# Distributed-Learning-Networking-Group/torchgpipe

Hardware: AMD Instinct MI355X
Metric: U-Net(5,64) GPipe training throughput (samples/sec) (higher is better)
Workload: dtype fp32; 1 GPU; model=U-Net(5,64), experiment=pipeline-1, global_batch=80, input=3x192x192, chunks=2, checkpoint=except_last, parallelism=pp1, transport=none, fused_cells=True, cell_streams=0, overlap_recompute=True, overlap_forward=True, graph_cells=False, hw_queues=4

## Files before the change

### torchgpipe_amd/csrc/bindings.cpp

```cpp
#include <algorithm>
#include <torch/extension.h>
#include <ATen/hip/HIPContext.h>
#include <ATen/hip/impl/HIPGuardImplMasqueradingAsCUDA.h>

#include <vector>

#include "kernels.h"

namespace tgpipe {
namespace {

hipStream_t stream_of(const at::Tensor& t) {
  return at::hip::getCurrentHIPStream(t.device().index()).stream();
}

const int64_t* rng_state(const c10::optional<at::Tensor>& rng, const at::Device& device) {
  if (!rng.has_value() || !rng->defined()) return nullptr;
  TORCH_CHECK(rng->is_cuda() && rng->device() == device && rng->scalar_type() == at::kLong &&
                  rng->is_contiguous() && rng->numel() == 2,
              "rng must be a contiguous int64 [2] (seed, offset) tensor on the op's device");
  return rng->data_ptr<int64_t>();
}

void check_f32_gpu(const at::Tensor& t, const char* name) {
  TORCH_CHECK(t.is_cuda(), name, " must be a GPU tensor");
  TORCH_CHECK(t.scalar_type() == at::kFloat, name, " must be float32");
  TORCH_CHECK(t.is_contiguous(), name, " must be contiguous");
}

std::vector<at::Tensor> dna_forward(const at::Tensor& x, double p, double eps, double slope,
                                    int64_t seed, int64_t offset, bool dropout,
                                    const c10::optional<at::Tensor>& rng) {
  check_f32_gpu(x, "x");
  TORCH_CHECK(x.dim() >= 3, "expected (N, C, *spatial) input");
  TORCH_CHECK(p >= 0.0 && p < 1.0, "dropout probability must be in [0, 1)");
  const int64_t planes = x.size(0) * x.size(1);
  const int64_t s = planes == 0 ? 0 : x.numel() / planes;
  c10::hip::HIPGuardMasqueradingAsCUDA guard(x.device());
  auto y = at::empty_like(x);
  auto opts = x.options();
  auto mean = at::empty({planes}, opts);
  auto rstd = at::empty({planes}, opts);
  auto scale = at::empty({planes}, opts);
  launch_dna_forward(x.data_ptr<float>(), y.data_ptr<float>(), mean.data_ptr<float>(),
                     rstd.data_ptr<float>(), scale.data_ptr<float>(), planes, s,
                     static_cast<float>(p), static_cast<float>(eps), static_cast<float>(slope),
                     static_cast<uint64_t>(seed), static_cast<uint64_t>(offset), dropout,
                     rng_state(rng, x.device()), stream_of(x));
  return {y, mean, rstd, scale};
}

at::Tensor dna_backward(const at::Tensor& dy_in, const at::Tensor& x, const at::Tensor& mean,
                        const at::Tensor& rstd, const at::Tensor& scale, double slope) {
  check_f32_gpu(x, "x");
  auto dy = dy_in.contiguous();
  check_f32_gpu(dy, "dy");
  TORCH_CHECK(dy.sizes() == x.sizes(), "dy and x must have the same shape");
  const int64_t planes = x.size(0) * x.size(1);
  const int64_t s = planes == 0 ? 0 : x.numel() / planes;
  TORCH_CHECK(mean.numel() == planes && rstd.numel() == planes && scale.numel() == planes,
              "saved statistics must have N*C elements");
  c10::hip::HIPGuardMasqueradingAsCUDA guard(x.device());
  auto dx = at::empty_like(x);
  launch_dna_backward(dy.data_ptr<float>(), x.data_ptr<float>(), mean.data_ptr<float>(),
                      rstd.data_ptr<float>(), scale.data_ptr<float>(), dx.data_ptr<float>(),
                      planes, s, static_cast<float>(slope), stream_of(x));
  return dx;
}

at::Tensor dropout(const at::Tensor& x_in, double p, int64_t seed, int64_t offset,
                   const c10::optional<at::Tensor>& rng) {
  auto x = x_in.contiguous();
  check_f32_gpu(x, "x");
  TORCH_CHECK(p >= 0.0 && p < 1.0, "dropout probability must be in [0, 1)");
  c10::hip::HIPGuardMasqueradingAsCUDA guard(x.device());
  auto y = at::empty_like(x);
  launch_dropout(x.data_ptr<float>(), y.data_ptr<float>(), x.numel(), static_cast<float>(p),
                 static_cast<uint64_t>(seed), static_cast<uint64_t>(offset),
                 rng_state(rng, x.device()), stream_of(x));
  return y;
}

at::Tensor philox_uniform(int64_t n, int64_t seed, int64_t offset, at::Device device,
                          const c10::optional<at::Tensor>& rng) {
  TORCH_CHECK(device.is_cuda(), "philox_uniform runs on the GPU");
  c10::hip::HIPGuardMasqueradingAsCUDA guard(device);
  auto out = at::empty({n}, at::TensorOptions().dtype(at::kFloat).device(device));
  launch_philox_uniform(out.data_ptr<float>(), n, static_cast<uint64_t>(seed),
                        static_cast<uint64_t>(offset), rng_state(rng, out.device()),
                        stream_of(out));
  return out;
}

void spin(int64_t ns, at::Device device) {
  TORCH_CHECK(device.is_cuda(), "spin runs on the GPU");
  c10::hip::HIPGuardMasqueradingAsCUDA guard(device);
  launch_spin(static_cast<uint64_t>(ns),
              at::hip::getCurrentHIPStream(device.index()).stream());
}

void copy_segments(at::TensorList srcs, at::TensorList dsts) {
  TORCH_CHECK(srcs.size() == dsts.size(), "srcs and dsts must pair up");
  if (srcs.empty()) return;
  const auto device = srcs[0].device();
  TORCH_CHECK(device.is_cuda(), "copy_segments runs on the GPU");
  c10::hip::HIPGuardMasqueradingAsCUDA guard(device);
  std::vector<Segment> segs;
  for (size_t i = 0; i < srcs.size(); ++i) {
    TORCH_CHECK(srcs[i].is_contiguous() && dsts[i].is_contiguous(), "segments must be contiguous");
    TORCH_CHECK(srcs[i].device() == device && dsts[i].device() == device,
                "segments must live on one device");
    const int64_t bytes = srcs[i].numel() * srcs[i].element_size();
    TORCH_CHECK(bytes == dsts[i].numel() * dsts[i].element_size(), "segment size mismatch");
    segs.push_back({srcs[i].data_ptr(), dsts[i].data_ptr(), bytes});
  }
  const hipStream_t stream = at::hip::getCurrentHIPStream(device.index()).stream();
  for (size_t i = 0; i < segs.size(); i += kMaxSegments) {
    const int count = static_cast<int>(std::min<size_t>(kMaxSegments, segs.size() - i));
    launch_segments_copy(segs.data() + i, count, stream);
  }
}

at::Tensor transform_out(const c10::optional<at::Tensor>& out, at::IntArrayRef shape,
                         const at::Tensor& like) {
  if (!out.has_value() || !out->defined()) return at::empty(shape, like.options());
  check_f32_gpu(*out, "out");
  TORCH_CHECK(out->sizes() == shape && out->device() == like.device(),
              "out must be the transform's shape on the weight's device");
  return *out;
}

at::Tensor wino_weight(const at::Tensor& w, bool flip, const c10::optional<at::Tensor>& out) {
  check_f32_gpu(w, "weight");
  TORCH_CHECK(w.dim() == 4 && w.size(2) == 3 && w.size(3) == 3, "weight must be [K][C][3][3]");
  const int64_t out_channels = flip ? w.size(1) : w.size(0);
  const int64_t red_channels = flip ? w.size(0) : w.size(1);
  c10::hip::HIPGuardMasqueradingAsCUDA guard(w.device());
  auto u = transform_out(
      out, {wino_pad_reduction(red_channels), wino_pad_output(out_channels), 16}, w);
  launch_wino_weight(w.data_ptr<float>(), u.data_ptr<float>(), out_channels, red_channels, flip,
                     stream_of(w));
  return u;
}

at::Tensor wino_conv(const at::Tensor& x_in, const at::Tensor& u,
                     const c10::optional<at::Tensor>& bias, int64_t out_channels,
                     int64_t variant, int64_t splits) {
  auto x = x_in.contiguous();
  check_f32_gpu(x, "x");
  check_f32_gpu(u, "u");
  TORCH_CHECK(x.dim() == 4, "x must be NCHW");
  const int64_t n = x.size(0), r = x.size(1), h = x.size(2), w = x.size(3);
  TORCH_CHECK(u.dim() == 3 && u.size(2) == 16 && u.size(0) == wino_pad_reduction(r) &&
                  u.size(1) == wino_pad_output(out_channels),
              "transformed weight does not match the input/output channels");
  TORCH_CHECK(u.device() == x.device(), "u must live on the input's device");
  TORCH_CHECK(n * ((h + 1) / 2) * ((w + 1) / 2) < (int64_t{1} << 31) * 32,
              "too many output tiles for one launch");
  TORCH_CHECK(r * h * w < (int64_t{1} << 31) && out_channels < (1 << 24),
              "plane too large for 32-bit channel offsets");
  const float* bptr = nullptr;
  if (bias.has_value() && bias->defined()) {
    check_f32_gpu(*bias, "bias");
    TORCH_CHECK(bias->numel() == out_channels, "bias must have K elements");
    bptr = bias->data_ptr<float>();
  }
  c10::hip::HIPGuardMasqueradingAsCUDA guard(x.device());
  TORCH_CHECK(variant >= -1 && variant <= 2, "variant must be -1 (auto), 0, 1 or 2");
  auto y = at::empty({n, out_channels, h, w}, x.options());
  if (y.numel() == 0) return y;
  const WinoPlan plan = wino_plan(n, r, h, w, out_channels, static_cast<int>(variant),
                                  static_cast<int>(splits));
  at::Tensor ws;
  if (plan.workspace > 0) ws = at::empty({plan.workspace}, x.options());
  launch_wino_conv(x.data_ptr<float>(), u.data_ptr<float>(), bptr, y.data_ptr<float>(),
                   plan.workspace > 0 ? ws.data_ptr<float>() : nullptr, n, r, h, w, out_channels,
                   plan, stream_of(x));
  return y;
}

at::Tensor wino4_weight(const at::Tensor& w, bool flip, const c10::optional<at::Tensor>& out) {
  check_f32_gpu(w, "weight");
  TORCH_CHECK(w.dim() == 4 && w.size(2) == 3 && w.size(3) == 3, "weight must be [K][C][3][3]");
  const int64_t out_channels = flip ? w.size(1) : w.size(0);
  const int64_t red_channels = flip ? w.size(0) : w.size(1);
  c10::hip::HIPGuardMasqueradingAsCUDA guard(w.device());
  auto u = transform_out(
      out, {wino4_pad_reduction(red_channels), wino4_pad_output(out_channels), 36}, w);
  launch_wino4_weight(w.data_ptr<float>(), u.data_ptr<float>(), out_channels, red_channels, flip,
                      stream_of(w));
  return u;
}

std::vector<int64_t> wino4_emu_weight_shape(int64_t out_channels, int64_t red_channels) {
  return {wino4_emu_pad_reduction(red_channels) / 16, wino4_pad_output(out_channels) / 64, 36,
          1024};
}

at::Tensor wino4_weight_emu(const at::Tensor& w, bool flip,
                            const c10::optional<at::Tensor>& out) {
  check_f32_gpu(w, "weight");
  TORCH_CHECK(w.dim() == 4 && w.size(2) == 3 && w.size(3) == 3, "weight must be [K][C][3][3]");
  const int64_t out_channels = flip ? w.size(1) : w.size(0);
  const int64_t red_channels = flip ? w.size(0) : w.size(1);
  c10::hip::HIPGuardMasqueradingAsCUDA guard(w.device());
  const auto wc = w.contiguous();
  auto u = transform_out(out, wino4_emu_weight_shape(out_channels, red_channels), w);
  TORCH_CHECK(u.is_contiguous(), "out must be contiguous");
  if (u.numel() == 0) return u;
  launch_wino4_emu_weight(wc.data_ptr<float>(), u.data_ptr<float>(), out_channels, red_channels,
                          flip, stream_of(w));
  return u;
}

at::Tensor wino4_conv(const at::Tensor& x_in, const at::Tensor& u,
                      const c10::optional<at::Tensor>& bias, int64_t out_channels,
                      int64_t variant, int64_t splits) {
  auto x = x_in.contiguous();
  check_f32_gpu(x, "x");
// ... 63 lines not shown
  auto dw = wgrad_destination(into, x, k, c);
  if (n == 0 || h == 0 || w == 0) return accum ? dw : dw.zero_();
  TORCH_CHECK(variant == -1 || variant == 0 || variant == 2, "variant must be -1, 0 or 2");
  const int64_t tiles = n * ((h + 1) / 2) * ((w + 1) / 2);
  int v = variant >= 0 ? static_cast<int>(variant) : (k <= 32 ? 0 : 2);
  if (v == 2 && tiles >= (int64_t{1} << 24)) v = 0;
  const int64_t steps = (tiles + 7) / 8;
  const int s = static_cast<int>(std::min<int64_t>(
      splits > 0 ? splits : wino_wgrad_splits(n, c, k, h, w, v), steps));
  at::Tensor ws;
  if (s > 1) ws = at::empty({s * k * c * 9}, x.options());
  launch_wino_wgrad(x.data_ptr<float>(), dy.data_ptr<float>(), dw.data_ptr<float>(),
                    s > 1 ? ws.data_ptr<float>() : nullptr, n, c, k, h, w, s, v, accum,
                    stream_of(x));
  return dw;
}

at::Tensor wino4_wgrad(const at::Tensor& x_in, const at::Tensor& dy_in, int64_t splits,
                       int64_t variant, const c10::optional<at::Tensor>& into) {
  auto x = x_in.contiguous();
  auto dy = dy_in.contiguous();
  check_f32_gpu(x, "x");
  check_f32_gpu(dy, "dy");
  TORCH_CHECK(x.dim() == 4 && dy.dim() == 4, "x and dy must be NCHW");
  const int64_t n = x.size(0), c = x.size(1), h = x.size(2), w = x.size(3), k = dy.size(1);
  TORCH_CHECK(dy.size(0) == n && dy.size(2) == h && dy.size(3) == w,
              "dy must be [N][K][H][W] of a 3x3/s1/p1 convolution of x");
  TORCH_CHECK(dy.device() == x.device(), "x and dy must share a device");
  c10::hip::HIPGuardMasqueradingAsCUDA guard(x.device());
  const bool accum = into.has_value();
  auto dw = wgrad_destination(into, x, k, c);
  if (n == 0 || h == 0 || w == 0 || c == 0 || k == 0) return accum ? dw : dw.zero_();
  TORCH_CHECK(wino4_wgrad_supported(n, c, k, h, w),
              "input too large for the F(4x4) weight-gradient kernel (needs < 1 GiB); "
              "use wino_wgrad");
  TORCH_CHECK(variant >= 0 && variant <= 3,
              "variant must be 0 (fused), 1 (non-fused), 2 (split-bf16 batched GEMM) or 3 (fused, "
              "x rows through LDS)");
  const WinoPlan plan = wino4_wgrad_plan(n, c, k, h, w, static_cast<int>(variant),
                                         static_cast<int>(splits));
  at::Tensor ws;
  if (plan.workspace > 0) ws = at::empty({plan.workspace}, x.options());
  launch_wino4_wgrad(x.data_ptr<float>(), dy.data_ptr<float>(), dw.data_ptr<float>(),
                     plan.workspace > 0 ? ws.data_ptr<float>() : nullptr, n, c, k, h, w, plan,
                     accum, stream_of(x));
  return dw;
}

at::Tensor bg_weight(const at::Tensor& w, bool flip, int64_t kind,
                     const c10::optional<at::Tensor>& out, int64_t emu) {
  check_f32_gpu(w, "weight");
  TORCH_CHECK(w.dim() == 4 && w.size(2) == 3 && w.size(3) == 3, "weight must be [K][C][3][3]");
  auto wc = w.contiguous();
  const int64_t out_channels = flip ? w.size(1) : w.size(0);
  const int64_t red_channels = flip ? w.size(0) : w.size(1);
  c10::hip::HIPGuardMasqueradingAsCUDA guard(w.device());
  TORCH_CHECK(kind == 4 || kind == 2, "kind must be 4 (F(4x4)) or 2 (F(2x2))");
  auto a =
      transform_out(out, {bg_weight_numel(out_channels, red_channels, static_cast<int>(kind),
                                          static_cast<int>(emu))}, w);
  launch_bg_weight(wc.data_ptr<float>(), a.data_ptr<float>(), out_channels, red_channels, flip,
                   static_cast<int>(kind), stream_of(w), static_cast<int>(emu));
  return a;
}

at::Tensor bg_conv(const at::Tensor& x_in, const at::Tensor& a,
                   const c10::optional<at::Tensor>& bias, int64_t out_channels, int64_t bn,
                   int64_t splits, int64_t kind, int64_t waves, int64_t sub, int64_t emu,
                   const c10::optional<at::Tensor>& stats) {
  auto x = x_in.contiguous();
  check_f32_gpu(x, "x");
  check_f32_gpu(a, "a");
  TORCH_CHECK(x.dim() == 4, "x must be NCHW");
  const int64_t n = x.size(0), r = x.size(1), h = x.size(2), w = x.size(3);
  TORCH_CHECK(kind == 4 || kind == 2, "kind must be 4 (F(4x4)) or 2 (F(2x2))");
  TORCH_CHECK(a.dim() == 1 && a.numel() == bg_weight_numel(out_channels, r, static_cast<int>(kind),
                                                           static_cast<int>(emu)),
              "batched-GEMM transformed weight does not match the input/output channels");
  TORCH_CHECK(a.device() == x.device(), "a must live on the input's device");
  TORCH_CHECK(wino4_supported(n, r, h, w, out_channels),
              "input too large for the F(4x4) kernels (needs < 1 GiB)");
  const float* bptr = nullptr;
  if (bias.has_value() && bias->defined()) {
    check_f32_gpu(*bias, "bias");
    TORCH_CHECK(bias->numel() == out_channels, "bias must have K elements");
    bptr = bias->data_ptr<float>();
  }
  c10::hip::HIPGuardMasqueradingAsCUDA guard(x.device());
  auto y = at::empty({n, out_channels, h, w}, x.options());
  if (n == 0 || h == 0 || w == 0 || out_channels == 0) return y;
  const BgPlan plan = bg_plan(n, r, h, w, out_channels, static_cast<int>(bn),
                              static_cast<int>(splits), static_cast<int>(kind),
                              static_cast<int>(waves), static_cast<int>(sub),
                              static_cast<int>(emu));
  TORCH_CHECK(plan.ksteps * 16 * plan.np < (int64_t{1} << 31) &&
                  plan.mp * plan.np < (int64_t{1} << 31),
              "operands too large for the batched-GEMM kernels");
  float* pm = nullptr;
  int ipg = 0;
  if (stats.has_value() && stats->defined()) {
    check_f32_gpu(*stats, "stats");
    ipg = bg_stats_ipg(n, h, w, static_cast<int>(kind));
    const int64_t groups = (n + ipg - 1) / ipg;
    TORCH_CHECK(stats->device() == x.device() && stats->is_contiguous() &&
                    stats->numel() == 2 * groups * out_channels,
                "stats must be a contiguous [2][ceil(n / bg_stats_ipg)][K] float32 tensor");
    pm = stats->data_ptr<float>();
  }
  auto ws = at::empty({plan.workspace}, x.options());
  launch_bg_conv(x.data_ptr<float>(), a.data_ptr<float>(), bptr, y.data_ptr<float>(),
                 ws.data_ptr<float>(), n, r, h, w, out_channels, plan, stream_of(x), pm,
                 pm == nullptr ? nullptr : pm + stats->numel() / 2, ipg);
  return y;
}

int64_t bg_stats_images(int64_t n, int64_t h, int64_t w, int64_t kind) {
  return bg_stats_ipg(n, h, w, static_cast<int>(kind));
}

int64_t wino4_splits(int64_t n, int64_t c, int64_t k, int64_t h, int64_t w, int64_t variant) {
  if (variant == 0) return wino4_wgrad_plan(n, c, k, h, w, 0, 0).splits;
  return wino4_plan(n, c, h, w, k, static_cast<int>(variant), 0).splits;
}

std::vector<int64_t> wino4_plan_info(int64_t n, int64_t c, int64_t k, int64_t h, int64_t w,
                                     int64_t variant, int64_t splits) {
  const WinoPlan p = wino4_plan(n, c, h, w, k, static_cast<int>(variant),
                                static_cast<int>(splits));
  return {p.variant, p.og, p.splits, p.workspace};
}

std::vector<int64_t> wino4_wgrad_plan_info(int64_t n, int64_t c, int64_t k, int64_t h, int64_t w,
                                           int64_t variant, int64_t splits) {
  const WinoPlan p = wino4_wgrad_plan(n, c, k, h, w, static_cast<int>(variant),
                                      static_cast<int>(splits));
  return {p.variant, p.splits, p.workspace};
}

std::vector<int64_t> bg_plan_info(int64_t n, int64_t c, int64_t k, int64_t h, int64_t w,
                                  int64_t bn, int64_t splits, int64_t kind, int64_t waves,
                                  int64_t sub, int64_t emu) {
  const BgPlan p = bg_plan(n, c, h, w, k, static_cast<int>(bn), static_cast<int>(splits),
                           static_cast<int>(kind), static_cast<int>(waves),
                           static_cast<int>(sub), static_cast<int>(emu));
  return {p.kind, p.emu ? 1 : 0, p.waves, p.bn, p.sub, p.splits, p.ksteps, p.mp, p.np,
          p.workspace};
}

}
}

TORCH_LIBRARY(tgpipe, m) {
  m.def("dna_forward(Tensor x, float p, float eps, float slope, int seed, int offset, "
        "bool dropout, Tensor? rng=None) -> Tensor[]");
  m.def("dna_backward(Tensor dy, Tensor x, Tensor mean, Tensor rstd, Tensor scale, "
        "float slope) -> Tensor");
  m.def("dropout(Tensor x, float p, int seed, int offset, Tensor? rng=None) -> Tensor");
  m.def("philox_uniform(int n, int seed, int offset, Device device, Tensor? rng=None) -> Tensor");
  m.def("spin(int ns, Device device) -> ()");
  m.def("copy_segments(Tensor[] srcs, Tensor(a!)[] dsts) -> ()");
  m.def("wino_weight(Tensor w, bool flip, Tensor? out=None) -> Tensor");
  m.def("wino_wgrad(Tensor x, Tensor dy, int splits=0, int variant=-1, Tensor? into=None) -> Tensor");
  m.def("wino_conv(Tensor x, Tensor u, Tensor? bias, int out_channels, int variant=-1, "
        "int splits=0) -> Tensor");
  m.def("wino4_weight(Tensor w, bool flip, Tensor? out=None) -> Tensor");
  m.def("wino4_weight_emu(Tensor w, bool flip, Tensor? out=None) -> Tensor");
  m.def("wino4_wgrad(Tensor x, Tensor dy, int splits=0, int variant=0, Tensor? into=None) -> Tensor");
  m.def("wino4_conv(Tensor x, Tensor u, Tensor? bias, int out_channels, int variant=-1, "
        "int splits=0) -> Tensor");
  m.def("bg_weight(Tensor w, bool flip, int kind=4, Tensor? out=None, int emu=-1) -> Tensor");
  m.def("wino4_splits(int n, int c, int k, int h, int w, int variant) -> int",
        &tgpipe::wino4_splits);
  m.def("bg_conv(Tensor x, Tensor a, Tensor? bias, int out_channels, int bn=0, int splits=0, "
        "int kind=4, int waves=0, int sub=0, int emu=-1, Tensor(b!)? stats=None) -> Tensor");
  m.def("wino4_plan_info(int n, int c, int k, int h, int w, int variant, int splits) -> int[]",
        &tgpipe::wino4_plan_info);
  m.def("wino4_wgrad_plan_info(int n, int c, int k, int h, int w, int variant, int splits) "
        "-> int[]", &tgpipe::wino4_wgrad_plan_info);
  m.def("bg_plan_info(int n, int c, int k, int h, int w, int bn, int splits, int kind, "
        "int waves, int sub, int emu) -> int[]", &tgpipe::bg_plan_info);
  m.def("bg_stats_images(int n, int h, int w, int kind) -> int", &tgpipe::bg_stats_images);
}

TORCH_LIBRARY_IMPL(tgpipe, CUDA, m) {
  m.impl("dna_forward", &tgpipe::dna_forward);
  m.impl("dna_backward", &tgpipe::dna_backward);
  m.impl("dropout", &tgpipe::dropout);
  m.impl("copy_segments", &tgpipe::copy_segments);
  m.impl("wino_weight", &tgpipe::wino_weight);
  m.impl("wino_conv", &tgpipe::wino_conv);
  m.impl("wino_wgrad", &tgpipe::wino_wgrad);
  m.impl("wino4_weight", &tgpipe::wino4_weight);
  m.impl("wino4_weight_emu", &tgpipe::wino4_weight_emu);
  m.impl("wino4_conv", &tgpipe::wino4_conv);
  m.impl("wino4_wgrad", &tgpipe::wino4_wgrad);
  m.impl("bg_weight", &tgpipe::bg_weight);
  m.impl("bg_conv", &tgpipe::bg_conv);
}

TORCH_LIBRARY_IMPL(tgpipe, CompositeExplicitAutograd, m) {
  m.impl("philox_uniform", &tgpipe::philox_uniform);
  m.impl("spin", &tgpipe::spin);
}

PYBIND11_MODULE(TORCH_EXTENSION_NAME, m) {
  m.doc() = "torchgpipe_amd native HIP kernels (gfx950)";
}
```

### torchgpipe_amd/csrc/kernels.h

```cpp
#pragma once
#include <hip/hip_runtime.h>
#include <stdint.h>

#include <vector>

namespace tgpipe {

void launch_dna_forward(const float* x, float* y, float* mean, float* rstd, float* scale,
                        int64_t planes, int64_t s, float p, float eps, float slope,
                        uint64_t seed, uint64_t offset, bool dropout, const int64_t* rng,
                        hipStream_t stream);

void launch_dna_backward(const float* dy, const float* x, const float* mean, const float* rstd,
                         const float* scale, float* dx, int64_t planes, int64_t s, float slope,
                         hipStream_t stream);

void launch_dropout(const float* x, float* y, int64_t n, float p, uint64_t seed, uint64_t offset,
                    const int64_t* rng, hipStream_t stream);

void launch_philox_uniform(float* out, int64_t n, uint64_t seed, uint64_t offset,
                           const int64_t* rng, hipStream_t stream);

void launch_spin(uint64_t ns, hipStream_t stream);

struct Segment {
  const void* src;
  void* dst;
  int64_t bytes;
};
constexpr int kMaxSegments = 16;
void launch_segments_copy(const Segment* segs, int count, hipStream_t stream);

int64_t wino_pad_reduction(int64_t r);
int64_t wino_pad_output(int64_t o);
void launch_wino_weight(const float* w, float* u, int64_t out_channels, int64_t red_channels,
                        bool flip, hipStream_t stream);
struct WinoPlan {
  int variant = 0;
  int splits = 1;
  int64_t workspace = 0;
  int og = 0;
};
WinoPlan wino_plan(int64_t n, int64_t red_channels, int64_t h, int64_t w, int64_t out_channels,
                   int variant, int splits);
void launch_wino_conv(const float* x, const float* u, const float* bias, float* y, float* ws,
                      int64_t n, int64_t red_channels, int64_t h, int64_t w, int64_t out_channels,
                      const WinoPlan& plan, hipStream_t stream);

int64_t wino4_pad_reduction(int64_t r);
int64_t wino4_pad_output(int64_t o);
bool wino4_supported(int64_t n, int64_t r, int64_t h, int64_t w, int64_t o);
void launch_wino4_weight(const float* w, float* u, int64_t out_channels, int64_t red_channels,
                         bool flip, hipStream_t stream);
bool wino4_variant_known(int variant);
bool wino4_variant_emu(int variant);
int64_t wino4_emu_pad_reduction(int64_t r);
int64_t wino4_emu_weight_numel(int64_t out_channels, int64_t red_channels);
void launch_wino4_emu_weight(const float* w, float* u, int64_t out_channels,
                             int64_t red_channels, bool flip, hipStream_t stream);
WinoPlan wino4_plan(int64_t n, int64_t red_channels, int64_t h, int64_t w, int64_t out_channels,
                    int variant, int splits);
void launch_wino4_conv(const float* x, const float* u, const float* bias, float* y, float* ws,
                       int64_t n, int64_t red_channels, int64_t h, int64_t w, int64_t out_channels,
                       const WinoPlan& plan, hipStream_t stream);

struct BgPlan {
  int kind = 4;
  int waves = 8;
  int bn = 64;
  int sub = 1;
  int splits = 1;
  bool emu = false;
  int64_t mp = 0, np = 0, ksteps = 0;
  int64_t workspace = 0;
};
bool bg_emu(int emu);
int bg_pick_bn(int64_t tiles, int kind, bool emu = false);
BgPlan bg_plan(int64_t n, int64_t red_channels, int64_t h, int64_t w, int64_t out_channels,
               int bn, int splits, int kind, int waves, int sub, int emu = -1);
int64_t bg_weight_numel(int64_t out_channels, int64_t red_channels, int kind, int emu = -1);
void launch_bg_weight(const float* w, float* a, int64_t out_channels, int64_t red_channels,
                      bool flip, int kind, hipStream_t stream, int emu = -1);
int bg_stats_ipg(int64_t n, int64_t h, int64_t w, int kind);
void launch_bg_conv(const float* x, const float* a, const float* bias, float* y, float* ws,
                    int64_t n, int64_t red_channels, int64_t h, int64_t w, int64_t out_channels,
                    const BgPlan& plan, hipStream_t stream, float* pm = nullptr,
                    float* pm2 = nullptr, int ipg = 0);


bool wino4_wgrad_supported(int64_t n, int64_t c, int64_t k, int64_t h, int64_t w);
WinoPlan wino4_wgrad_plan(int64_t n, int64_t c, int64_t k, int64_t h, int64_t w, int variant,
                          int splits);
void launch_wino4_wgrad(const float* x, const float* dy, float* dw, float* ws, int64_t n,
                        int64_t c, int64_t k, int64_t h, int64_t w, const WinoPlan& plan,
                        bool accum, hipStream_t stream);

int wino_wgrad_splits(int64_t n, int64_t c, int64_t k, int64_t h, int64_t w, int variant);
void launch_wino_wgrad(const float* x, const float* dy, float* dw, float* ws, int64_t n,
                       int64_t c, int64_t k, int64_t h, int64_t w, int splits, int variant,
                       bool accum, hipStream_t stream);


struct ConvGemmTail {
  const float* gamma = nullptr;
  const float* beta = nullptr;
  const float* mean = nullptr;
  const float* var = nullptr;
  const float* add = nullptr;
  float eps = 0.f;
  int relu_out = 0;
};
struct ConvGemmGeo {
  int n, ci, h, w;
  int co, ho, wo;
  int co_total, co_off;
  int kh, kw, sh, sw, ph, pw;
  int oh, ow;
  bool relu;
  bool a_t = false;
  bool phase = false;
  int zh = 0, zw = 0, dy0 = 0, dx0 = 0;
  bool fill = false;
  bool a_split = false;
  ConvGemmTail tail;
};
struct ConvGemmPhase {
  ConvGemmGeo geo;
  int th0, tw0;
};
bool conv_gemm_phased(const ConvGemmGeo& g);
constexpr int kConvGemmMaxPhases = 4;
struct ConvGemmPlan;
void launch_conv_gemm_phases(const float* a, const int64_t* a_off, const float* b,
                             const float* x_mask, float* out, const ConvGemmPhase* phases,
                             int count, const ConvGemmPlan& plan, bool accumulate,
                             int64_t a_bytes, int64_t b_bytes, hipStream_t stream);
int env_int(const char* name, int fallback);
std::vector<ConvGemmPhase> conv_gemm_phases(const ConvGemmGeo& g);
struct ConvGemmPlan {
  int cfg = 1;
  int splits = 1;
  int col_width = 128;
  int col_blocks = 0;
  bool scatter = false;
};
ConvGemmPlan conv_gemm_plan(int mode, const ConvGemmGeo& g);
std::vector<ConvGemmPlan> conv_gemm_candidates(int mode, const ConvGemmGeo& g);
int64_t conv_gemm_workspace(int mode, const ConvGemmGeo& g, const ConvGemmPlan& plan);
void launch_conv_gemm(int mode, const float* a, const float* b, const float* x_mask, float* out,
                      float* part_mean, float* part_m2, const ConvGemmGeo& g,
                      const ConvGemmPlan& plan, bool accumulate, float* ws, int64_t a_bytes,
                      int64_t b_bytes, hipStream_t stream);
bool conv_gemm_emu_cfg(int cfg);
int conv_precision(int level);
int conv_precision_level();
class ConvPrecisionPin {
 public:
  explicit ConvPrecisionPin(int level);
  ~ConvPrecisionPin();
  ConvPrecisionPin(const ConvPrecisionPin&) = delete;
  ConvPrecisionPin& operator=(const ConvPrecisionPin&) = delete;

 private:
  int saved_;
};
void launch_conv_gemm_presplit(const float* w, void* out, int M, int K, int taps,
                               bool transposed, hipStream_t stream);
void launch_conv_gemm_wgrad_slab(const float* a, const float* b, float* slab,
// ... 94 lines not shown
```

### torchgpipe_amd/csrc/kernels.hip

```cpp
#include "kernels.h"
#include "philox.h"

#include <hip/hip_runtime.h>
#include <math.h>

namespace tgpipe {

namespace {

constexpr int kWave = 64;

__device__ __forceinline__ float wave_sum(float v) {
#pragma unroll
  for (int o = kWave / 2; o > 0; o >>= 1) v += __shfl_xor(v, o, kWave);
  return v;
}

template <int GROUP>
__device__ __forceinline__ float group_sum_in_wave(float v) {
#pragma unroll
  for (int o = GROUP / 2; o > 0; o >>= 1) v += __shfl_xor(v, o, kWave);
  return v;
}

inline int ceil_div(int64_t a, int64_t b) { return static_cast<int>((a + b - 1) / b); }

template <int GROUP>
constexpr int kPlaneBlock = GROUP >= 256 ? GROUP : 256;

template <int GROUP, int V, bool VEC>
struct PlaneTile {
  static constexpr int kBlock = kPlaneBlock<GROUP>;
  static constexpr int kPlanesPerBlock = kBlock / GROUP;
  static constexpr int kCap = GROUP * V * 4;

  __device__ static __forceinline__ int64_t index(int t, int k, int j) {
    return VEC ? static_cast<int64_t>(k * GROUP + t) * 4 + j
               : static_cast<int64_t>(k * 4 + j) * GROUP + t;
  }

  __device__ static __forceinline__ void load(const float* __restrict__ p, int t, int64_t s,
                                              bool active, float (&r)[V * 4]) {
#pragma unroll
    for (int k = 0; k < V; ++k) {
      if (VEC) {
        const int64_t idx = index(t, k, 0);
        float4 v = (active && idx < s) ? *reinterpret_cast<const float4*>(p + idx)
                                       : make_float4(0, 0, 0, 0);
        r[k * 4 + 0] = v.x;
        r[k * 4 + 1] = v.y;
        r[k * 4 + 2] = v.z;
        r[k * 4 + 3] = v.w;
      } else {
#pragma unroll
        for (int j = 0; j < 4; ++j) {
          const int64_t idx = index(t, k, j);
          r[k * 4 + j] = (active && idx < s) ? p[idx] : 0.f;
        }
      }
    }
  }

  __device__ static __forceinline__ void store(float* __restrict__ p, int t, int64_t s,
                                               bool active, const float (&r)[V * 4]) {
    if (!active) return;
#pragma unroll
    for (int k = 0; k < V; ++k) {
      if (VEC) {
        const int64_t idx = index(t, k, 0);
        if (idx < s)
          *reinterpret_cast<float4*>(p + idx) =
              make_float4(r[k * 4 + 0], r[k * 4 + 1], r[k * 4 + 2], r[k * 4 + 3]);
      } else {
#pragma unroll
        for (int j = 0; j < 4; ++j) {
          const int64_t idx = index(t, k, j);
          if (idx < s) p[idx] = r[k * 4 + j];
        }
      }
    }
  }

  __device__ static __forceinline__ bool valid(int t, int k, int j, int64_t s) {
    return index(t, k, j) < s;
  }

  __device__ static __forceinline__ float reduce(float v, float* lds) {
    if (GROUP <= kWave) return group_sum_in_wave<GROUP>(v);
    v = wave_sum(v);
    const int wave = threadIdx.x / kWave;
    if ((threadIdx.x & (kWave - 1)) == 0) lds[wave] = v;
    __syncthreads();
    float total = 0.f;
#pragma unroll
    for (int w = 0; w < GROUP / kWave; ++w) total += lds[w];
    __syncthreads();
    return total;
  }
};

__device__ __forceinline__ void philox_resolve(const int64_t* __restrict__ rng, uint64_t& seed,
                                               uint64_t& offset) {
  if (rng != nullptr) {
    seed = static_cast<uint64_t>(rng[0]);
    offset += static_cast<uint64_t>(rng[1]);
  }
}

__device__ __forceinline__ float plane_dropout_scale(int64_t plane, float p, uint64_t seed,
                                                     uint64_t offset, bool dropout) {
  if (!dropout) return 1.f;
  const float u = philox_uniform(philox4x32_10(static_cast<uint64_t>(plane), offset, seed).v[0]);
  return u >= p ? 1.f / (1.f - p) : 0.f;
}

template <int GROUP, int V, bool VEC>
__global__ __launch_bounds__(kPlaneBlock<GROUP>) void dna_forward_kernel(
    const float* __restrict__ x, float* __restrict__ y, float* __restrict__ mean_out,
    float* __restrict__ rstd_out, float* __restrict__ scale_out, int64_t planes, int64_t s,
    float p, float eps, float slope, uint64_t seed, uint64_t offset, bool dropout,
    const int64_t* __restrict__ rng) {
  using T = PlaneTile<GROUP, V, VEC>;
  philox_resolve(rng, seed, offset);
  __shared__ float lds[T::kBlock / kWave];
  const int t = threadIdx.x % GROUP;
  const int64_t plane = static_cast<int64_t>(blockIdx.x) * T::kPlanesPerBlock + threadIdx.x / GROUP;
  const bool active = plane < planes;
  const float* xp = x + (active ? plane : 0) * s;

  float r[V * 4];
  T::load(xp, t, s, active, r);

  float acc = 0.f;
#pragma unroll
  for (int e = 0; e < V * 4; ++e) acc += r[e];
  const float inv_s = 1.f / static_cast<float>(s);
  const float mean = T::reduce(acc, lds) * inv_s;

  float sq = 0.f;
#pragma unroll
  for (int k = 0; k < V; ++k)
#pragma unroll
    for (int j = 0; j < 4; ++j) {
      const float d = T::valid(t, k, j, s) ? r[k * 4 + j] - mean : 0.f;
      sq += d * d;
    }
  const float var = T::reduce(sq, lds) * inv_s;

  const float scale = plane_dropout_scale(plane, p, seed, offset, dropout);
  const float rstd = rsqrtf(scale * scale * var + eps);
  const float mul = scale * rstd;
#pragma unroll
  for (int e = 0; e < V * 4; ++e) {
    const float z = (r[e] - mean) * mul;
    r[e] = z > 0.f ? z : z * slope;
  }
  T::store(y + (active ? plane : 0) * s, t, s, active, r);
  if (active && t == 0) {
    mean_out[plane] = mean;
    rstd_out[plane] = rstd;
    scale_out[plane] = scale;
  }
}

template <int GROUP, int V, bool VEC>
__global__ __launch_bounds__(kPlaneBlock<GROUP>) void dna_backward_kernel(
    const float* __restrict__ dy, const float* __restrict__ x, const float* __restrict__ mean_in,
    const float* __restrict__ rstd_in, const float* __restrict__ scale_in, float* __restrict__ dx,
    int64_t planes, int64_t s, float slope) {
  using T = PlaneTile<GROUP, V, VEC>;
  __shared__ float lds[T::kBlock / kWave];
  const int t = threadIdx.x % GROUP;
  const int64_t plane = static_cast<int64_t>(blockIdx.x) * T::kPlanesPerBlock + threadIdx.x / GROUP;
  const bool active = plane < planes;
  const int64_t base = (active ? plane : 0) * s;

  const float mean = active ? mean_in[plane] : 0.f;
  const float rstd = active ? rstd_in[plane] : 0.f;
  const float scale = active ? scale_in[plane] : 0.f;
  const float mul = scale * rstd;

  float z[V * 4];
  float g[V * 4];
  T::load(x + base, t, s, active, z);
  T::load(dy + base, t, s, active, g);

  float sg = 0.f, sgz = 0.f;
#pragma unroll
  for (int e = 0; e < V * 4; ++e) {
    z[e] = (z[e] - mean) * mul;
    g[e] = z[e] > 0.f ? g[e] : g[e] * slope;
    sg += g[e];
    sgz += g[e] * z[e];
  }
  const float inv_s = 1.f / static_cast<float>(s);
  const float mg = T::reduce(sg, lds) * inv_s;
  const float mgz = T::reduce(sgz, lds) * inv_s;
#pragma unroll
  for (int e = 0; e < V * 4; ++e) g[e] = mul * (g[e] - mg - z[e] * mgz);
  T::store(dx + base, t, s, active, g);
}

constexpr int kBigGroup = 1024;

__global__ __launch_bounds__(kBigGroup) void dna_forward_big_kernel(
    const float* __restrict__ x, float* __restrict__ y, float* __restrict__ mean_out,
    float* __restrict__ rstd_out, float* __restrict__ scale_out, int64_t s, float p, float eps,
    float slope, uint64_t seed, uint64_t offset, bool dropout, const int64_t* __restrict__ rng) {
  __shared__ float lds[kBigGroup / kWave];
  philox_resolve(rng, seed, offset);
  using T = PlaneTile<kBigGroup, 1, false>;
  const int64_t plane = blockIdx.x;
  const float* xp = x + plane * s;
  float acc = 0.f;
  for (int64_t i = threadIdx.x; i < s; i += kBigGroup) acc += xp[i];
  const float inv_s = 1.f / static_cast<float>(s);
  const float mean = T::reduce(acc, lds) * inv_s;
  float sq = 0.f;
  for (int64_t i = threadIdx.x; i < s; i += kBigGroup) {
    const float d = xp[i] - mean;
    sq += d * d;
  }
  const float var = T::reduce(sq, lds) * inv_s;
  const float scale = plane_dropout_scale(plane, p, seed, offset, dropout);
  const float rstd = rsqrtf(scale * scale * var + eps);
  const float mul = scale * rstd;
  float* yp = y + plane * s;
  for (int64_t i = threadIdx.x; i < s; i += kBigGroup) {
    const float z = (xp[i] - mean) * mul;
    yp[i] = z > 0.f ? z : z * slope;
  }
  if (threadIdx.x == 0) {
    mean_out[plane] = mean;
    rstd_out[plane] = rstd;
    scale_out[plane] = scale;
  }
}

__global__ __launch_bounds__(kBigGroup) void dna_backward_big_kernel(
    const float* __restrict__ dy, const float* __restrict__ x, const float* __restrict__ mean_in,
    const float* __restrict__ rstd_in, const float* __restrict__ scale_in, float* __restrict__ dx,
    int64_t s, float slope) {
  __shared__ float lds[kBigGroup / kWave];
  using T = PlaneTile<kBigGroup, 1, false>;
  const int64_t plane = blockIdx.x;
  const float mean = mean_in[plane];
  const float mul = scale_in[plane] * rstd_in[plane];
  const float* xp = x + plane * s;
  const float* gp = dy + plane * s;
  float sg = 0.f, sgz = 0.f;
  for (int64_t i = threadIdx.x; i < s; i += kBigGroup) {
    const float z = (xp[i] - mean) * mul;
    const float g = z > 0.f ? gp[i] : gp[i] * slope;
    sg += g;
    sgz += g * z;
  }
  const float inv_s = 1.f / static_cast<float>(s);
  const float mg = T::reduce(sg, lds) * inv_s;
  const float mgz = T::reduce(sgz, lds) * inv_s;
  float* dp = dx + plane * s;
  for (int64_t i = threadIdx.x; i < s; i += kBigGroup) {
    const float z = (xp[i] - mean) * mul;
    const float g = z > 0.f ? gp[i] : gp[i] * slope;
    dp[i] = mul * (g - mg - z * mgz);
  }
}

__global__ __launch_bounds__(256) void dropout_kernel(const float* __restrict__ x,
                                                      float* __restrict__ y, int64_t n, float p,
                                                      uint64_t seed, uint64_t offset, bool vec,
                                                      const int64_t* __restrict__ rng) {
  philox_resolve(rng, seed, offset);
  const float scale = 1.f / (1.f - p);
  const int64_t quads = (n + 3) / 4;
  for (int64_t q = static_cast<int64_t>(blockIdx.x) * blockDim.x + threadIdx.x; q < quads;
       q += static_cast<int64_t>(gridDim.x) * blockDim.x) {
    const PhiloxOut r = philox4x32_10(static_cast<uint64_t>(q), offset, seed);
    const int64_t e0 = q * 4;
    if (vec && e0 + 3 < n) {
      float4 v = *reinterpret_cast<const float4*>(x + e0);
      v.x = philox_uniform(r.v[0]) >= p ? v.x * scale : 0.f;
      v.y = philox_uniform(r.v[1]) >= p ? v.y * scale : 0.f;
      v.z = philox_uniform(r.v[2]) >= p ? v.z * scale : 0.f;
      v.w = philox_uniform(r.v[3]) >= p ? v.w * scale : 0.f;
      *reinterpret_cast<float4*>(y + e0) = v;
    } else {
      for (int j = 0; j < 4 && e0 + j < n; ++j)
        y[e0 + j] = philox_uniform(r.v[j]) >= p ? x[e0 + j] * scale : 0.f;
    }
  }
}

__global__ __launch_bounds__(256) void philox_uniform_kernel(float* __restrict__ out, int64_t n,
                                                             uint64_t seed, uint64_t offset,
                                                             const int64_t* __restrict__ rng) {
  philox_resolve(rng, seed, offset);
  const int64_t quads = (n + 3) / 4;
  for (int64_t q = static_cast<int64_t>(blockIdx.x) * blockDim.x + threadIdx.x; q < quads;
       q += static_cast<int64_t>(gridDim.x) * blockDim.x) {
    const PhiloxOut r = philox4x32_10(static_cast<uint64_t>(q), offset, seed);
    for (int j = 0; j < 4 && q * 4 + j < n; ++j) out[q * 4 + j] = philox_uniform(r.v[j]);
  }
}

__global__ void spin_kernel(uint64_t ticks) {
  const uint64_t t0 = __builtin_amdgcn_s_memrealtime();
  const uint64_t limit = ticks < 6000000000ull ? ticks : 6000000000ull;
  while (__builtin_amdgcn_s_memrealtime() - t0 < limit) __builtin_amdgcn_s_sleep(8);
}

struct SegmentTable {
  Segment seg[kMaxSegments];
};

__global__ __launch_bounds__(256) void segments_copy_kernel(SegmentTable table) {
  const Segment sg = table.seg[blockIdx.y];
  const uintptr_t a = reinterpret_cast<uintptr_t>(sg.src) | reinterpret_cast<uintptr_t>(sg.dst);
  const int64_t stride = static_cast<int64_t>(gridDim.x) * blockDim.x;
  const int64_t tid = static_cast<int64_t>(blockIdx.x) * blockDim.x + threadIdx.x;
  if ((a & 15) == 0) {
    const int64_t nvec = sg.bytes / 16;
    const uint4* s = reinterpret_cast<const uint4*>(sg.src);
    uint4* d = reinterpret_cast<uint4*>(sg.dst);
    for (int64_t i = tid; i < nvec; i += stride) d[i] = s[i];
    const int64_t tail = nvec * 16;
    const char* sb = reinterpret_cast<const char*>(sg.src);
    char* db = reinterpret_cast<char*>(sg.dst);
    for (int64_t i = tail + tid; i < sg.bytes; i += stride) db[i] = sb[i];
  } else {
    const char* sb = reinterpret_cast<const char*>(sg.src);
    char* db = reinterpret_cast<char*>(sg.dst);
    for (int64_t i = tid; i < sg.bytes; i += stride) db[i] = sb[i];
  }
}

template <int GROUP, int V, bool VEC>
void dna_fwd_launch(const float* x, float* y, float* mean, float* rstd, float* scale,
                    int64_t planes, int64_t s, float p, float eps, float slope, uint64_t seed,
                    uint64_t offset, bool dropout, const int64_t* rng, hipStream_t stream) {
  using T = PlaneTile<GROUP, V, VEC>;
  const int grid = ceil_div(planes, T::kPlanesPerBlock);
  hipLaunchKernelGGL((dna_forward_kernel<GROUP, V, VEC>), dim3(grid), dim3(T::kBlock), 0, stream,
                     x, y, mean, rstd, scale, planes, s, p, eps, slope, seed, offset, dropout,
                     rng);
}

template <int GROUP, int V, bool VEC>
void dna_bwd_launch(const float* dy, const float* x, const float* mean, const float* rstd,
                    const float* scale, float* dx, int64_t planes, int64_t s, float slope,
                    hipStream_t stream) {
  using T = PlaneTile<GROUP, V, VEC>;
  const int grid = ceil_div(planes, T::kPlanesPerBlock);
  hipLaunchKernelGGL((dna_backward_kernel<GROUP, V, VEC>), dim3(grid), dim3(T::kBlock), 0,
                     stream, dy, x, mean, rstd, scale, dx, planes, s, slope);
}

#define TGPIPE_DNA_DISPATCH(LAUNCH, VEC, ...)                      \
  if (s <= 16 * 1 * 4) {                                           \
    LAUNCH<16, 1, VEC>(__VA_ARGS__);                               \
  } else if (s <= 64 * 1 * 4) {                                    \
    LAUNCH<64, 1, VEC>(__VA_ARGS__);                               \
  } else if (s <= 64 * 3 * 4) {                                    \
    LAUNCH<64, 3, VEC>(__VA_ARGS__);                               \
  } else if (s <= 64 * 9 * 4) {                                    \
    LAUNCH<64, 9, VEC>(__VA_ARGS__);                               \
  } else if (s <= 256 * 9 * 4) {                                   \
    LAUNCH<256, 9, VEC>(__VA_ARGS__);                              \
  } else {                                                         \
    LAUNCH<1024, 9, VEC>(__VA_ARGS__);                             \
  }

}

constexpr int64_t kDnaMaxTile = 1024 * 9 * 4;

void launch_dna_forward(const float* x, float* y, float* mean, float* rstd, float* scale,
                        int64_t planes, int64_t s, float p, float eps, float slope,
                        uint64_t seed, uint64_t offset, bool dropout, const int64_t* rng,
                        hipStream_t stream) {
  if (planes == 0 || s == 0) return;
  if (s > kDnaMaxTile) {
    hipLaunchKernelGGL(dna_forward_big_kernel, dim3(static_cast<unsigned>(planes)),
                       dim3(kBigGroup), 0, stream, x, y, mean, rstd, scale, s, p, eps, slope,
                       seed, offset, dropout, rng);
    return;
  }
  const bool vec = (s % 4 == 0) && (((reinterpret_cast<uintptr_t>(x) |
                                      reinterpret_cast<uintptr_t>(y)) & 15) == 0);
  if (vec) {
    TGPIPE_DNA_DISPATCH(dna_fwd_launch, true, x, y, mean, rstd, scale, planes, s, p, eps, slope,
                        seed, offset, dropout, rng, stream)
  } else {
    TGPIPE_DNA_DISPATCH(dna_fwd_launch, false, x, y, mean, rstd, scale, planes, s, p, eps,
                        slope, seed, offset, dropout, rng, stream)
  }
}

void launch_dna_backward(const float* dy, const float* x, const float* mean, const float* rstd,
                         const float* scale, float* dx, int64_t planes, int64_t s, float slope,
                         hipStream_t stream) {
  if (planes == 0 || s == 0) return;
  if (s > kDnaMaxTile) {
    hipLaunchKernelGGL(dna_backward_big_kernel, dim3(static_cast<unsigned>(planes)),
                       dim3(kBigGroup), 0, stream, dy, x, mean, rstd, scale, dx, s, slope);
    return;
  }
  const bool vec = (s % 4 == 0) && (((reinterpret_cast<uintptr_t>(x) |
                                      reinterpret_cast<uintptr_t>(dy) |
                                      reinterpret_cast<uintptr_t>(dx)) & 15) == 0);
  if (vec) {
    TGPIPE_DNA_DISPATCH(dna_bwd_launch, true, dy, x, mean, rstd, scale, dx, planes, s, slope,
                        stream)
  } else {
    TGPIPE_DNA_DISPATCH(dna_bwd_launch, false, dy, x, mean, rstd, scale, dx, planes, s, slope,
                        stream)
  }
}

void launch_dropout(const float* x, float* y, int64_t n, float p, uint64_t seed, uint64_t offset,
                    const int64_t* rng, hipStream_t stream) {
  if (n == 0) return;
  const int64_t quads = (n + 3) / 4;
  int64_t grid = (quads + 255) / 256;
  if (grid > 2048) grid = 2048;
  const bool vec = ((reinterpret_cast<uintptr_t>(x) | reinterpret_cast<uintptr_t>(y)) & 15) == 0;
  hipLaunchKernelGGL(dropout_kernel, dim3(static_cast<unsigned>(grid)), dim3(256), 0, stream, x,
                     y, n, p, seed, offset, vec, rng);
}

void launch_philox_uniform(float* out, int64_t n, uint64_t seed, uint64_t offset,
                           const int64_t* rng, hipStream_t stream) {
  if (n == 0) return;
  int64_t grid = ((n + 3) / 4 + 255) / 256;
  if (grid > 2048) grid = 2048;
  hipLaunchKernelGGL(philox_uniform_kernel, dim3(static_cast<unsigned>(grid)), dim3(256), 0,
                     stream, out, n, seed, offset, rng);
}

void launch_spin(uint64_t ns, hipStream_t stream) {
  hipLaunchKernelGGL(spin_kernel, dim3(1), dim3(1), 0, stream, ns / 10);
}

void launch_segments_copy(const Segment* segs, int count, hipStream_t stream) {
  if (count <= 0) return;
  SegmentTable table{};
  int64_t largest = 0;
  for (int i = 0; i < count && i < kMaxSegments; ++i) {
    table.seg[i] = segs[i];
    if (segs[i].bytes > largest) largest = segs[i].bytes;
  }
  int64_t grid = (largest / 16 + 255) / 256;
  if (grid < 1) grid = 1;
  if (grid > 1024) grid = 1024;
  const int n = count < kMaxSegments ? count : kMaxSegments;
  hipLaunchKernelGGL(segments_copy_kernel, dim3(static_cast<unsigned>(grid), n), dim3(256), 0,
                     stream, table);
}

}
```

Before: 715.5 samples/sec.

## Add persistent double-buffered DNA forward and dropout-skipping DNA backward kernels

The forward dropout-norm-activation path gets a persistent-grid kernel for full vectorized tiles. It is sized from occupancy and prefetches the next plane's tile into registers while the current one is reduced and normalized, hiding load latency. The backward path gets a kernel that skips loading x and dy for planes whose dropout scale is zero and writes zeros directly. Both become the default (variant -1), and the old kernels stay reachable via variant 0. The cost is doubled register tiles in the forward, which may lower occupancy, plus an occupancy query on first use.

New measurement: 719.1 samples/sec (median of 6 runs). Within noise of the previous version (+0.5%).

```diff
diff --git a/torchgpipe_amd/csrc/bindings.cpp b/torchgpipe_amd/csrc/bindings.cpp
--- a/torchgpipe_amd/csrc/bindings.cpp
+++ b/torchgpipe_amd/csrc/bindings.cpp
@@ -30,7 +30,7 @@
 
 std::vector<at::Tensor> dna_forward(const at::Tensor& x, double p, double eps, double slope,
                                     int64_t seed, int64_t offset, bool dropout,
-                                    const c10::optional<at::Tensor>& rng) {
+                                    const c10::optional<at::Tensor>& rng, int64_t variant) {
   check_f32_gpu(x, "x");
   TORCH_CHECK(x.dim() >= 3, "expected (N, C, *spatial) input");
   TORCH_CHECK(p >= 0.0 && p < 1.0, "dropout probability must be in [0, 1)");
@@ -46,12 +46,13 @@
                      rstd.data_ptr<float>(), scale.data_ptr<float>(), planes, s,
                      static_cast<float>(p), static_cast<float>(eps), static_cast<float>(slope),
                      static_cast<uint64_t>(seed), static_cast<uint64_t>(offset), dropout,
-                     rng_state(rng, x.device()), stream_of(x));
+                     rng_state(rng, x.device()), stream_of(x), static_cast<int>(variant));
   return {y, mean, rstd, scale};
 }
 
 at::Tensor dna_backward(const at::Tensor& dy_in, const at::Tensor& x, const at::Tensor& mean,
-                        const at::Tensor& rstd, const at::Tensor& scale, double slope) {
+                        const at::Tensor& rstd, const at::Tensor& scale, double slope,
+                        int64_t variant) {
   check_f32_gpu(x, "x");
   auto dy = dy_in.contiguous();
   check_f32_gpu(dy, "dy");
@@ -64,7 +65,8 @@
   auto dx = at::empty_like(x);
   launch_dna_backward(dy.data_ptr<float>(), x.data_ptr<float>(), mean.data_ptr<float>(),
                       rstd.data_ptr<float>(), scale.data_ptr<float>(), dx.data_ptr<float>(),
-                      planes, s, static_cast<float>(slope), stream_of(x));
+                      planes, s, static_cast<float>(slope), stream_of(x),
+                      static_cast<int>(variant));
   return dx;
 }
 
@@ -434,9 +436,9 @@
 
 TORCH_LIBRARY(tgpipe, m) {
   m.def("dna_forward(Tensor x, float p, float eps, float slope, int seed, int offset, "
-        "bool dropout, Tensor? rng=None) -> Tensor[]");
+        "bool dropout, Tensor? rng=None, int variant=-1) -> Tensor[]");
   m.def("dna_backward(Tensor dy, Tensor x, Tensor mean, Tensor rstd, Tensor scale, "
-        "float slope) -> Tensor");
+        "float slope, int variant=-1) -> Tensor");
   m.def("dropout(Tensor x, float p, int seed, int offset, Tensor? rng=None) -> Tensor");
   m.def("philox_uniform(int n, int seed, int offset, Device device, Tensor? rng=None) -> Tensor");
   m.def("spin(int ns, Device device) -> ()");
diff --git a/torchgpipe_amd/csrc/kernels.h b/torchgpipe_amd/csrc/kernels.h
--- a/torchgpipe_amd/csrc/kernels.h
+++ b/torchgpipe_amd/csrc/kernels.h
@@ -9,11 +9,11 @@
 void launch_dna_forward(const float* x, float* y, float* mean, float* rstd, float* scale,
                         int64_t planes, int64_t s, float p, float eps, float slope,
                         uint64_t seed, uint64_t offset, bool dropout, const int64_t* rng,
-                        hipStream_t stream);
+                        hipStream_t stream, int variant = -1);
 
 void launch_dna_backward(const float* dy, const float* x, const float* mean, const float* rstd,
                          const float* scale, float* dx, int64_t planes, int64_t s, float slope,
-                         hipStream_t stream);
+                         hipStream_t stream, int variant = -1);
 
 void launch_dropout(const float* x, float* y, int64_t n, float p, uint64_t seed, uint64_t offset,
                     const int64_t* rng, hipStream_t stream);
diff --git a/torchgpipe_amd/csrc/kernels.hip b/torchgpipe_amd/csrc/kernels.hip
--- a/torchgpipe_amd/csrc/kernels.hip
+++ b/torchgpipe_amd/csrc/kernels.hip
@@ -3,6 +3,8 @@
 
 #include <hip/hip_runtime.h>
 #include <math.h>
+
+#include <stdexcept>
 
 namespace tgpipe {
 
@@ -59,6 +61,27 @@
         }
       }
     }
+  }
+
+  __device__ static __forceinline__ void load_full(const float* __restrict__ p, int t,
+                                                   float (&r)[V * 4]) {
+    static_assert(VEC, "full tiles are read in 16-byte slots");
+#pragma unroll
+    for (int k = 0; k < V; ++k) {
+      const float4 v = *reinterpret_cast<const float4*>(p + static_cast<uint32_t>(index(t, k, 0)));
+      r[k * 4 + 0] = v.x;
+      r[k * 4 + 1] = v.y;
+      r[k * 4 + 2] = v.z;
+      r[k * 4 + 3] = v.w;
+    }
+  }
+
+  __device__ static __forceinline__ void store_full(float* __restrict__ p, int t,
+                                                    const float (&r)[V * 4]) {
+#pragma unroll
+    for (int k = 0; k < V; ++k)
+      *reinterpret_cast<float4*>(p + static_cast<uint32_t>(index(t, k, 0))) =
+          make_float4(r[k * 4 + 0], r[k * 4 + 1], r[k * 4 + 2], r[k * 4 + 3]);
   }
 
   __device__ static __forceinline__ void store(float* __restrict__ p, int t, int64_t s,
@@ -198,6 +221,131 @@
   const float mgz = T::reduce(sgz, lds) * inv_s;
 #pragma unroll
   for (int e = 0; e < V * 4; ++e) g[e] = mul * (g[e] - mg - z[e] * mgz);
+  T::store(dx + base, t, s, active, g);
+}
+
+template <int GROUP>
+__global__ __launch_bounds__(kPlaneBlock<GROUP>) void dna_forward_pipe_kernel(
+    const float* __restrict__ x, float* __restrict__ y, float* __restrict__ mean_out,
+    float* __restrict__ rstd_out, float* __restrict__ scale_out, int64_t planes, float p,
+    float eps, float slope, uint64_t seed, uint64_t offset, bool dropout,
+    const int64_t* __restrict__ rng) {
+#pragma clang fp contract(off)
+  constexpr int V = 9;
+  using T = PlaneTile<GROUP, V, true>;
+  constexpr int64_t s = T::kCap;
+  philox_resolve(rng, seed, offset);
+  __shared__ float lds[T::kBlock / kWave];
+  const int t = threadIdx.x % GROUP;
+  const int sub = threadIdx.x / GROUP;
+  const float inv_s = 1.f / static_cast<float>(s);
+
+  auto plane_of = [&](int64_t b) -> int64_t {
+    return __builtin_amdgcn_readfirstlane(static_cast<int>(b * T::kPlanesPerBlock + sub));
+  };
+  auto fetch = [&](int64_t b, float (&r)[V * 4]) {
+    const int64_t plane = plane_of(b);
+    T::load_full(x + (plane < planes ? plane : 0) * s, t, r);
+  };
+  auto finish = [&](int64_t b, float (&r)[V * 4]) {
+    const int64_t plane = plane_of(b);
+    const bool active = T::kPlanesPerBlock == 1 || plane < planes;
+    float acc = 0.f;
+#pragma unroll
+    for (int e = 0; e < V * 4; ++e) acc += r[e];
+    const float total = T::reduce(acc, lds);
+    const float mean = total * inv_s;
+
+    float sq = __builtin_fmaf(-inv_s, total, r[1]);
+    sq *= sq;
+#pragma unroll
+    for (int e = 0; e < V * 4; ++e) {
+      if (e == 1) continue;
+      const float d = __builtin_fmaf(-inv_s, total, r[e]);
+      sq = __builtin_fmaf(d, d, sq);
+    }
+    const float var = T::reduce(sq, lds) * inv_s;
+
+    const float scale = plane_dropout_scale(plane, p, seed, offset, dropout);
+    const float rstd = rsqrtf(__builtin_fmaf(var, scale * scale, eps));
+    const float mul = scale * rstd;
+#pragma unroll
+    for (int e = 0; e < V * 4; ++e) {
+      const float z = (r[e] - mean) * mul;
+      r[e] = z > 0.f ? z : z * slope;
+    }
+    if (!active) return;
+    T::store_full(y + plane * s, t, r);
+    if (t == 0) {
+      mean_out[plane] = mean;
+      rstd_out[plane] = rstd;
+      scale_out[plane] = scale;
+    }
+  };
+
+  float ra[V * 4], rb[V * 4];
+  const int64_t blocks = (planes + T::kPlanesPerBlock - 1) / T::kPlanesPerBlock;
+  const int64_t step = gridDim.x;
+  int64_t b = blockIdx.x;
+  fetch(b, ra);
+  while (true) {
+    fetch(b + step, rb);
+    finish(b, ra);
+    b += step;
+    if (b >= blocks) break;
+    fetch(b + step, ra);
+    finish(b, rb);
+    b += step;
+    if (b >= blocks) break;
+  }
+}
+
+template <int GROUP, int V, bool VEC>
+__global__ __launch_bounds__(kPlaneBlock<GROUP>) void dna_backward_skip_kernel(
+    const float* __restrict__ dy, const float* __restrict__ x, const float* __restrict__ mean_in,
+    const float* __restrict__ rstd_in, const float* __restrict__ scale_in, float* __restrict__ dx,
+    int64_t planes, int64_t s, float slope) {
+#pragma clang fp contract(off)
+  using T = PlaneTile<GROUP, V, VEC>;
+  __shared__ float lds[T::kBlock / kWave];
+  const int t = threadIdx.x % GROUP;
+  const int64_t plane = static_cast<int64_t>(blockIdx.x) * T::kPlanesPerBlock + threadIdx.x / GROUP;
+  const bool active = plane < planes;
+  const int64_t base = (active ? plane : 0) * s;
+
+  const float mean = active ? mean_in[plane] : 0.f;
+  const float rstd = active ? rstd_in[plane] : 0.f;
+  const float scale = active ? scale_in[plane] : 0.f;
+  const float mul = scale * rstd;
+  const bool live = scale != 0.f;
+
+  float z[V * 4];
+  float g[V * 4];
+  if (GROUP >= kWave && !live) {
+#pragma unroll
+    for (int e = 0; e < V * 4; ++e) g[e] = 0.f;
+    T::store(dx + base, t, s, active, g);
+    return;
+  }
+  T::load(x + base, t, s, live, z);
+  T::load(dy + base, t, s, live, g);
+
+  float sg = 0.f, sgz = 0.f;
+#pragma unroll
+  for (int e = 0; e < V * 4; ++e) {
+    z[e] = (z[e] - mean) * mul;
+    g[e] = z[e] > 0.f ? g[e] : g[e] * slope;
+    sg += g[e];
+    sgz = VEC ? sgz + g[e] * z[e] : __builtin_fmaf(g[e], z[e], sgz);
+  }
+  const float inv_s = 1.f / static_cast<float>(s);
+  const float mg = T::reduce(sg, lds) * inv_s;
+  const float mgz = T::reduce(sgz, lds) * inv_s;
+#pragma unroll
+  for (int e = 0; e < V * 4; ++e) {
+    const float u = mul * __builtin_fmaf(-z[e], mgz, g[e] - mg);
+    g[e] = (GROUP >= kWave || live) ? u : 0.f;
+  }
   T::store(dx + base, t, s, active, g);
 }
 
@@ -355,6 +503,48 @@
                      stream, dy, x, mean, rstd, scale, dx, planes, s, slope);
 }
 
+template <typename K>
+int resident_blocks(K kernel, int block) {
+  int dev = 0, cus = 0, per_cu = 0;
+  if (hipGetDevice(&dev) != hipSuccess ||
+      hipDeviceGetAttribute(&cus, hipDeviceAttributeMultiprocessorCount, dev) != hipSuccess ||
+      hipOccupancyMaxActiveBlocksPerMultiprocessor(&per_cu, kernel, block, 0) != hipSuccess ||
+      cus * per_cu < 1)
+    throw std::runtime_error("dna_forward: cannot size the persistent grid");
+  return cus * per_cu;
+}
+
+template <int GROUP, int V, bool VEC>
+void dna_fwd_pipe_launch(const float* x, float* y, float* mean, float* rstd, float* scale,
+                         int64_t planes, int64_t s, float p, float eps, float slope,
+                         uint64_t seed, uint64_t offset, bool dropout, const int64_t* rng,
+                         hipStream_t stream) {
+  using T = PlaneTile<GROUP, V, VEC>;
+  if constexpr (VEC && V == 9) {
+    if (s == T::kCap) {
+      static const int resident = resident_blocks(dna_forward_pipe_kernel<GROUP>, T::kBlock);
+      int grid = ceil_div(planes, T::kPlanesPerBlock);
+      if (grid > resident) grid = resident;
+      hipLaunchKernelGGL(dna_forward_pipe_kernel<GROUP>, dim3(grid), dim3(T::kBlock), 0, stream,
+                         x, y, mean, rstd, scale, planes, p, eps, slope, seed, offset, dropout,
+                         rng);
+      return;
+    }
+  }
+  dna_fwd_launch<GROUP, V, VEC>(x, y, mean, rstd, scale, planes, s, p, eps, slope, seed, offset,
+                                dropout, rng, stream);
+}
+
+template <int GROUP, int V, bool VEC>
+void dna_bwd_skip_launch(const float* dy, const float* x, const float* mean, const float* rstd,
+                         const float* scale, float* dx, int64_t planes, int64_t s, float slope,
+                         hipStream_t stream) {
+  using T = PlaneTile<GROUP, V, VEC>;
+  const int grid = ceil_div(planes, T::kPlanesPerBlock);
+  hipLaunchKernelGGL((dna_backward_skip_kernel<GROUP, V, VEC>), dim3(grid), dim3(T::kBlock), 0,
+                     stream, dy, x, mean, rstd, scale, dx, planes, s, slope);
+}
+
 #define TGPIPE_DNA_DISPATCH(LAUNCH, VEC, ...)                      \
   if (s <= 16 * 1 * 4) {                                           \
     LAUNCH<16, 1, VEC>(__VA_ARGS__);                               \
@@ -377,7 +567,8 @@
 void launch_dna_forward(const float* x, float* y, float* mean, float* rstd, float* scale,
                         int64_t planes, int64_t s, float p, float eps, float slope,
                         uint64_t seed, uint64_t offset, bool dropout, const int64_t* rng,
-                        hipStream_t stream) {
+                        hipStream_t stream, int variant) {
+  if (variant < -1 || variant > 0) throw std::runtime_error("dna_forward: variant -1 or 0");
   if (planes == 0 || s == 0) return;
   if (s > kDnaMaxTile) {
     hipLaunchKernelGGL(dna_forward_big_kernel, dim3(static_cast<unsigned>(planes)),
@@ -387,18 +578,26 @@
   }
   const bool vec = (s % 4 == 0) && (((reinterpret_cast<uintptr_t>(x) |
                                       reinterpret_cast<uintptr_t>(y)) & 15) == 0);
-  if (vec) {
-    TGPIPE_DNA_DISPATCH(dna_fwd_launch, true, x, y, mean, rstd, scale, planes, s, p, eps, slope,
-                        seed, offset, dropout, rng, stream)
+#define TGPIPE_DNA_FORWARD(LAUNCH)                                                            \
+  if (vec) {                                                                                  \
+    TGPIPE_DNA_DISPATCH(LAUNCH, true, x, y, mean, rstd, scale, planes, s, p, eps, slope, seed, \
+                        offset, dropout, rng, stream)                                         \
+  } else {                                                                                    \
+    TGPIPE_DNA_DISPATCH(LAUNCH, false, x, y, mean, rstd, scale, planes, s, p, eps, slope,     \
+                        seed, offset, dropout, rng, stream)                                   \
+  }
+  if (variant == 0) {
+    TGPIPE_DNA_FORWARD(dna_fwd_launch)
   } else {
-    TGPIPE_DNA_DISPATCH(dna_fwd_launch, false, x, y, mean, rstd, scale, planes, s, p, eps,
-                        slope, seed, offset, dropout, rng, stream)
-  }
+    TGPIPE_DNA_FORWARD(dna_fwd_pipe_launch)
+  }
+#undef TGPIPE_DNA_FORWARD
 }
 
 void launch_dna_backward(const float* dy, const float* x, const float* mean, const float* rstd,
                          const float* scale, float* dx, int64_t planes, int64_t s, float slope,
-                         hipStream_t stream) {
+                         hipStream_t stream, int variant) {
+  if (variant < -1 || variant > 0) throw std::runtime_error("dna_backward: variant -1 or 0");
   if (planes == 0 || s == 0) return;
   if (s > kDnaMaxTile) {
     hipLaunchKernelGGL(dna_backward_big_kernel, dim3(static_cast<unsigned>(planes)),
@@ -408,13 +607,19 @@
   const bool vec = (s % 4 == 0) && (((reinterpret_cast<uintptr_t>(x) |
                                       reinterpret_cast<uintptr_t>(dy) |
                                       reinterpret_cast<uintptr_t>(dx)) & 15) == 0);
-  if (vec) {
-    TGPIPE_DNA_DISPATCH(dna_bwd_launch, true, dy, x, mean, rstd, scale, dx, planes, s, slope,
-                        stream)
+#define TGPIPE_DNA_BACKWARD(LAUNCH)                                                          \
+  if (vec) {                                                                                 \
+    TGPIPE_DNA_DISPATCH(LAUNCH, true, dy, x, mean, rstd, scale, dx, planes, s, slope, stream) \
+  } else {                                                                                   \
+    TGPIPE_DNA_DISPATCH(LAUNCH, false, dy, x, mean, rstd, scale, dx, planes, s, slope,       \
+                        stream)                                                              \
+  }
+  if (variant == 0) {
+    TGPIPE_DNA_BACKWARD(dna_bwd_launch)
   } else {
-    TGPIPE_DNA_DISPATCH(dna_bwd_launch, false, dy, x, mean, rstd, scale, dx, planes, s, slope,
-                        stream)
-  }
+    TGPIPE_DNA_BACKWARD(dna_bwd_skip_launch)
+  }
+#undef TGPIPE_DNA_BACKWARD
 }
 
 void launch_dropout(const float* x, float* y, int64_t n, float p, uint64_t seed, uint64_t offset,
```
